# PufferAI/PufferLib

Hardware: AMD Instinct MI355X
Metric: env steps/sec end-to-end PPO (rollout+GAE+update), 4096 envs (higher is better)
Workload: dtype f32; 1 GPU; squared d=3 nt=1, 4096 envs/GPU x 128 steps, obs 49->64 f32 rows, MLP 128, 4 minibatches x 4 epochs, bptt 16 (BASELINE configs[1]); global_batch=524288, parallelism=dp1

## Files before the change

include/pufferlib_amd.h:

```cpp
#ifndef PUFFERLIB_AMD_H
#define PUFFERLIB_AMD_H
#include <stddef.h>
#include <stdint.h>

#ifdef __cplusplus
extern "C" {
#endif

typedef void *pfa_stream_t;

int pfa_version(void);
const char *pfa_last_error(void);

int pfa_timing_enable(int mode);
int pfa_timing_select(const char *kernel);
int pfa_timing_stride(int every);
int pfa_timing_reset(void);
int pfa_timing_read(const char *kernel, int64_t *launches_host, double *total_ms_host);

size_t pfa_gae_workspace_bytes(int64_t n);
int pfa_gae_f32(const float *dones, const float *values, const float *rewards, float *advantages,
                float *returns, int64_t n, float gamma, float gae_lambda, void *workspace,
                pfa_stream_t stream);
int pfa_gae_sums_supported(int64_t n, int32_t num_envs, int32_t num_minibatches, int32_t bptt_horizon);
size_t pfa_gae_sums_workspace_bytes(int64_t n, int32_t num_minibatches);
int pfa_gae_sums_f32(const float *dones, const float *values, const float *rewards, float *advantages, float *returns,
                     int64_t n, float gamma, float gae_lambda, int32_t num_envs, int32_t num_minibatches, int32_t bptt_horizon,
                     double *adv_stats, double *ev4, double *zero8, void *workspace, pfa_stream_t stream);
int32_t pfa_gae_halo_rows(float gamma, float gae_lambda);
int pfa_gae_halo_publish(const float *dones, const float *values, const float *rewards, int64_t n, float gamma, float gae_lambda,
                         const double *extra, int32_t n_extra, double *out, int32_t rank, int32_t world, pfa_stream_t stream);
int pfa_gae_halo_unpack(const double *gathered, int32_t rank, int32_t world, int64_t n, float gamma, float gae_lambda, float *dones,
                        float *values, float *rewards, pfa_stream_t stream);
int pfa_gae_halo_f32(const float *dones, const float *values, const float *rewards, float *advantages, float *returns, int64_t n,
                     int32_t halo_len, float gamma, float gae_lambda, int32_t num_envs, int32_t num_minibatches, int32_t bptt_horizon,
                     double *adv_stats, double *ev4, double *zero8, void *workspace, pfa_stream_t stream);
int pfa_gae_shard_pass2(const float *dones, const float *values, const float *rewards, float *advantages,
                        float *returns, int64_t n, int has_next, float gamma, float gae_lambda,
                        const void *workspace, const double *carry_in, pfa_stream_t stream);
int pfa_gae_shard_publish(const float *dones, const float *values, const float *rewards, int64_t n, float gamma, float gae_lambda,
                          void *workspace, const double *extra, int32_t n_extra, double *out, int32_t rank, int32_t world,
                          pfa_stream_t stream);
int pfa_gae_shard_fold(const double *gathered, int32_t rank, int32_t world, int64_t n, float gamma, float gae_lambda, void *workspace,
                       float *dones, float *values, float *rewards, double *carry_out, pfa_stream_t stream);


typedef struct {
    int32_t num_envs;
    int32_t distance_to_target;
    int32_t num_targets;
    int32_t obs_stride;
    int32_t tape_rounds;
} pfa_squared_config;

size_t pfa_squared_state_bytes(const pfa_squared_config *cfg);
int pfa_squared_async_reset(void *state, const pfa_squared_config *cfg, int64_t seed, float *obs,
                            float *rewards, uint8_t *terminals, uint8_t *truncations, uint8_t *masks,
                            pfa_stream_t stream);
int pfa_squared_fill_tape(void *state, const pfa_squared_config *cfg, int32_t rounds, pfa_stream_t stream);
int pfa_squared_send(void *state, const pfa_squared_config *cfg, const int64_t *actions, float *obs,
                     float *rewards, uint8_t *terminals, uint8_t *truncations, uint8_t *masks,
// ... 481 lines not shown
```

pufferlib_amd/_lib.py:

```python
import ctypes as C
import os
import subprocess

from .exceptions import ExtensionError

HERE = os.path.dirname(os.path.abspath(__file__))
REPO = os.path.dirname(HERE)
CSRC = os.path.join(HERE, 'csrc')
LIB_DIR = os.path.join(HERE, '_lib')
LIB_PATH = os.path.join(LIB_DIR, 'libpufferlib_amd.so')
SOURCES = ['common.cpp', 'dist.cpp', 'p2p.hip', 'gae.hip', 'squared.hip', 'pixel_squared.hip', 'rollout.hip', 'ppo_update.hip', 'lstm.hip', 'gemm.hip', 'lstm_fused.hip', 'lstm_seq.hip', 'stochastic.hip', 'memory.hip', 'bandit.hip', 'multiagent.hip', 'spaces.hip', 'synthetic.hip', 'tabular.hip', 'cartpole.hip', 'acrobot.hip', 'nativize.hip', 'igemm.hip', 'cnn_heads.hip', 'general.hip', 'ppo_wide.hip']
HEADERS = sorted(f for f in os.listdir(CSRC) if f.endswith('.hpp')) + [os.path.join('..', '..', 'include', 'pufferlib_amd.h')]


def _stale():
    if not os.path.exists(LIB_PATH):
        return True
    t = os.path.getmtime(LIB_PATH)
    deps = [os.path.join(CSRC, f) for f in SOURCES + HEADERS]
    return any(os.path.exists(d) and os.path.getmtime(d) > t for d in deps)


def source_hash():
    import hashlib
# ... 114 lines not shown


class Experience(C.Structure):
    _fields_ = [('obs', C.c_void_p), ('actions', C.c_void_p), ('logprobs', C.c_void_p), ('values', C.c_void_p),
                ('rewards', C.c_void_p), ('dones', C.c_void_p), ('advantages', C.c_void_p), ('returns', C.c_void_p),
                ('horizon_T', C.c_int32)]


class ReduceJob(C.Structure):
    _fields_ = [('kind', C.c_int32), ('splits', C.c_int32), ('mo', C.c_int32), ('no', C.c_int32), ('partial', C.c_void_p), ('c', C.c_void_p),
                ('ldc', C.c_int64), ('c2', C.c_void_p), ('ldc2', C.c_int64), ('nb', C.c_int32), ('reserved', C.c_int32)]


class PpoHparams(C.Structure):
    _fields_ = [('clip_coef', C.c_float), ('vf_clip_coef', C.c_float), ('vf_coef', C.c_float), ('ent_coef', C.c_float),
                ('norm_adv', C.c_int32), ('clip_vloss', C.c_int32), ('num_minibatches', C.c_int32),
                ('bptt_horizon', C.c_int32)]


P = C.c_void_p
_SIGNATURES = {
    'pfa_version': (C.c_int, []),
    'pfa_last_error': (C.c_char_p, []),
    'pfa_timing_enable': (C.c_int, [C.c_int]),
    'pfa_timing_select': (C.c_int, [C.c_char_p]),
    'pfa_timing_stride': (C.c_int, [C.c_int]),
    'pfa_timing_reset': (C.c_int, []),
    'pfa_timing_read': (C.c_int, [C.c_char_p, C.POINTER(C.c_int64), C.POINTER(C.c_double)]),
    'pfa_gae_workspace_bytes': (C.c_size_t, [C.c_int64]),
    'pfa_gae_f32': (C.c_int, [P, P, P, P, P, C.c_int64, C.c_float, C.c_float, P, P]),
    'pfa_gae_sums_supported': (C.c_int, [C.c_int64, C.c_int32, C.c_int32, C.c_int32]),
    'pfa_gae_sums_workspace_bytes': (C.c_size_t, [C.c_int64, C.c_int32]),
    'pfa_gae_sums_f32': (C.c_int, [P, P, P, P, P, C.c_int64, C.c_float, C.c_float, C.c_int32, C.c_int32, C.c_int32, P, P, P, P, P]),
    'pfa_gae_halo_rows': (C.c_int32, [C.c_float, C.c_float]),
    'pfa_gae_halo_publish': (C.c_int, [P, P, P, C.c_int64, C.c_float, C.c_float, P, C.c_int32, P, C.c_int32, C.c_int32, P]),
    'pfa_gae_halo_unpack': (C.c_int, [P, C.c_int32, C.c_int32, C.c_int64, C.c_float, C.c_float, P, P, P, P]),
    'pfa_gae_halo_f32': (C.c_int, [P, P, P, P, P, C.c_int64, C.c_int32, C.c_float, C.c_float, C.c_int32, C.c_int32, C.c_int32, P, P, P, P, P]),
    'pfa_gae_shard_pass2': (C.c_int, [P, P, P, P, P, C.c_int64, C.c_int, C.c_float, C.c_float, P, P, P]),
    'pfa_gae_shard_publish': (C.c_int, [P, P, P, C.c_int64, C.c_float, C.c_float, P, P, C.c_int32, P, C.c_int32, C.c_int32, P]),
    'pfa_gae_shard_fold': (C.c_int, [P, C.c_int32, C.c_int32, C.c_int64, C.c_float, C.c_float, P, P, P, P, P, P]),
    'pfa_train_ev_sums': (C.c_int, [C.POINTER(Experience), C.c_int64, C.c_int32, P, P, P]),
    'pfa_train_log_pack': (C.c_int, [P, P, P, P]),
    'pfa_squared_state_bytes': (C.c_size_t, [C.POINTER(SquaredConfig)]),
    'pfa_squared_async_reset': (C.c_int, [P, C.POINTER(SquaredConfig), C.c_int64, P, P, P, P, P, P]),
    'pfa_squared_fill_tape': (C.c_int, [P, C.POINTER(SquaredConfig), C.c_int32, P]),
    'pfa_squared_send': (C.c_int, [P, C.POINTER(SquaredConfig), P, P, P, P, P, P, P]),
    'pfa_squared_episode_stats': (C.c_int, [P, C.POINTER(SquaredConfig), P, C.c_int32, P]),
    'pfa_squared_last_infos': (C.c_int, [P, C.POINTER(SquaredConfig), P, P, P, P, P]),
    'pfa_squared_debug_targets': (C.c_int, [P, C.POINTER(SquaredConfig), P, P]),
    'pfa_squared_debug_stream_pos': (C.c_int, [P, C.POINTER(SquaredConfig), P, P]),
    'pfa_pixel_squared_state_bytes': (C.c_size_t, [C.POINTER(SquaredConfig), C.POINTER(PixelConfig)]),
    'pfa_pixel_squared_async_reset': (C.c_int, [P, C.POINTER(SquaredConfig), C.POINTER(PixelConfig), C.c_int64, P, P, P, P, P, P]),
    'pfa_pixel_squared_send': (C.c_int, [P, C.POINTER(SquaredConfig), C.POINTER(PixelConfig), P, P, P, P, P, P, P]),
    'pfa_mlp_param_count': (C.c_int64, [C.POINTER(MlpDims)]),
    'pfa_mlp_forward_sample': (C.c_int, [P, C.c_int64, P, C.POINTER(MlpDims), P, C.POINTER(NoiseKey), C.c_int64,
                                         P, P, P, P, P]),
    'pfa_philox_exp_noise': (C.c_int, [P, C.c_int64, C.c_int64, C.c_int32, C.POINTER(NoiseKey), C.c_int64, P]),
    'pfa_rollout_mlp_squared': (C.c_int, [P, C.POINTER(SquaredConfig), P, C.POINTER(MlpDims), C.POINTER(Experience),
                                          P, C.POINTER(NoiseKey), C.c_int64, P, P, P, P, P, P]),
    'pfa_mlp_view_supported': (C.c_int, [C.POINTER(MlpView)]),
    'pfa_ppo_wide_supported': (C.c_int, [C.POINTER(MlpView)]),
    'pfa_ppo_wide_workspace_bytes': (C.c_size_t, [C.POINTER(MlpView)]),
    'pfa_ppo_wide_grad': (C.c_int, [C.POINTER(Experience), C.c_int64, C.c_int32, C.POINTER(MlpView), C.POINTER(MlpView), P, C.POINTER(PpoHparams), P,
                                    C.c_int64, P, P]),
    'pfa_mlp_view_forward_sample': (C.c_int, [P, C.c_int64, C.POINTER(MlpView), P, C.POINTER(NoiseKey), C.c_int64, P, P, P, P, P]),
    'pfa_rollout_mlp_view_squared': (C.c_int, [P, C.POINTER(SquaredConfig), C.POINTER(MlpView), C.POINTER(Experience), P, C.POINTER(NoiseKey),
# ... 227 lines not shown
```

pufferlib_amd/clean_pufferl.py:

```python
import ctypes as C
import os
import random
import time
from collections import deque
from threading import Thread

import numpy as np
import torch

from . import _lib, readback, utils
from . import dist as pdist
from .cleanrl import Policy, RecurrentPolicy, _weights_changed, reads_frames, route
from .models import FlatParams
from .namespace import namespace
from .vector import Frames, PixelSquared, Spaces, Squared, Stochastic, _DeviceVecEnv


def seed_everything(seed, torch_deterministic=True):
    random.seed(seed)
    np.random.seed(seed)
    if seed is not None:
        torch.manual_seed(seed)
    torch.backends.cudnn.deterministic = torch_deterministic

# ... 526 lines not shown
            data._gae_done = _gae_key(data)
        if readback.eager():
            data._rb_eval.resolve()
    return stats, infos


def _early_gae():
    return os.environ.get('PFA_EARLY_GAE', '1') != '0'


def _ev_with_gae(data, world):
    return not (getattr(data, 'arrival_values', None) is not None and _cfg(data.config, 'async_store', 'balanced') == 'reference')


def _fused_sums_ok(data, world=1):
    config, experience = data.config, data.experience
    return (_ev_with_gae(data, world)
            and bool(_lib.lib().pfa_gae_sums_supported(experience.batch_size, experience.num_envs, experience.num_minibatches,
                                                       int(config.bptt_horizon))))


def _gae_key(data):
    config, ex = data.config, data.experience
    rdv = getattr(ex, '_rdv', None)
    ver = rdv._version if rdv is not None else (ex.rewards._version, ex.dones._version, ex.values._version)
    ptrs = tuple(int(getattr(ex, k).data_ptr()) for k in ('rewards', 'dones', 'values', 'advantages', 'returns'))
    return (ver, ptrs, ex.batch_size, float(config.gamma), float(config.gae_lambda), ex.num_envs, ex.num_minibatches,
            int(config.bptt_horizon), bool(config.norm_adv))


def _launch_gae_sums(data):
    config, experience = data.config, data.experience
    nmb = experience.num_minibatches
    _lib.check(_lib.lib().pfa_gae_sums_f32(
        _lib.ptr(experience.dones), _lib.ptr(experience.values), _lib.ptr(experience.rewards), _lib.ptr(experience.advantages),
        _lib.ptr(experience.returns), experience.batch_size, float(config.gamma), float(config.gae_lambda), experience.num_envs, nmb,
        int(config.bptt_horizon), _lib.ptr(data.adv_stats), C.c_void_p(data.dp_sums.data_ptr() + 16 * nmb), _lib.ptr(data.loss_acc),
        _lib.ptr(data.workspace), _lib.stream_handle()), 'gae_sums')


def _all_reduce(data, buf, what):
    if data.native_dp:
        L = _lib.lib()
        fn = L.pfa_dist_all_reduce_f64 if buf.dtype == torch.float64 else L.pfa_dist_all_reduce_f32
        _lib.check(fn(_lib.ptr(buf), buf.numel(), _lib.stream_handle()), what)
    elif data.world_size > 1:
        _dist()[0].all_reduce(buf)


def _publish_gae(data, extra=None):
    config, ex = data.config, data.experience
    L, B, stream = _lib.lib(), ex.batch_size, _lib.stream_handle()
    _, rank, world = _dist()
    gamma, lam = float(config.gamma), float(config.gae_lambda)
    n_extra = 0 if extra is None else extra.numel()
    H = int(L.pfa_gae_halo_rows(gamma, lam))
    if getattr(ex, '_rdv', None) is None or ex._rdv.shape[1] < B + H:
        H = 0
    size = n_extra + (3 * world * min(B, H) if H else 6 * world)
    if data._dp_eval is None or data._dp_eval.numel() != size:
        data._dp_eval = torch.zeros(size, dtype=torch.float64, device=ex.device)
    buf = data._dp_eval
    rows = (_lib.ptr(ex.dones), _lib.ptr(ex.values), _lib.ptr(ex.rewards))
    if H:
        _lib.check(L.pfa_gae_halo_publish(*rows, B, gamma, lam, _lib.ptr(extra), n_extra, _lib.ptr(buf), rank, world, stream), 'gae halo publish')
    else:
        _lib.check(L.pfa_gae_shard_publish(*rows, B, gamma, lam, _lib.ptr(data.gae_ws), _lib.ptr(extra), n_extra, _lib.ptr(buf), rank, world,
                                           stream), 'gae publish')
    _all_reduce(data, buf, 'stats + gae all-reduce')
    data._gae_published = (H, n_extra)
    return buf[:n_extra]
# ... 310 lines not shown
```

pufferlib_amd/csrc/gae.hip:

```cpp
#include <cmath>
#include <cstdlib>

#include "common.hpp"

#define PFA_GAE_FP _Pragma("clang fp contract(off)")

namespace pfa {

constexpr int kGaeThreads = 256;
constexpr int kGaeItems = 8;
constexpr int kGaeBlock = kGaeThreads * kGaeItems;

struct Affine {
    double c, d;
};

__device__ __forceinline__ Affine compose(const Affine &outer, const Affine &inner) {
    return {outer.c * inner.c, outer.d + outer.c * inner.d};
}

__device__ __forceinline__ Affine shfl_down_affine(const Affine &a, int off) {
    return {__shfl_down(a.c, off, 64), __shfl_down(a.d, off, 64)};
}

struct GaeItems {
    float v[kGaeItems + 1], r[kGaeItems + 1], d[kGaeItems + 1];
};

__device__ __forceinline__ void gae_load(const float *dones, const float *values, const float *rewards, long long s,
                                         long long n, GaeItems &it) {
#pragma unroll
    for (int i = 0; i <= kGaeItems; ++i) {
        const long long t = s + i;
        const bool ok = t < n;
        it.v[i] = ok ? values[t] : 0.0f;
        it.r[i] = ok ? rewards[t] : 0.0f;
        it.d[i] = ok ? dones[t] : 0.0f;
    }
}

__device__ __forceinline__ Affine gae_thread_map(const GaeItems &it, long long s, long long n, float gamma, float lam,
                                                 bool pin_last) {
    PFA_GAE_FP
    Affine f = {1.0, 0.0};
#pragma unroll
    for (int i = kGaeItems - 1; i >= 0; --i) {
        const long long t = s + i;
        if (t >= n) continue;
        if (t == n - 1 && pin_last) {
            f = {0.0, 0.0};
            continue;
        }
        const float nnt = 1.0f - it.d[i + 1];
        const float delta = (it.r[i + 1] + (gamma * it.v[i + 1]) * nnt) - it.v[i];
        const float coef = (gamma * lam) * nnt;
        f = compose({(double)coef, (double)delta}, f);
    }
    return f;
}

template <int NT = kGaeThreads>
__device__ __forceinline__ void block_suffix_scan(Affine &mine, Affine &after, Affine *sh) {
    const int lane = lane_id(), wv = wave_id();
// ... 48 lines not shown
        if (lane == 0) s_carry = f.c * (carry_in ? *carry_in : 0.0) + f.d;
    }
    const long long s = (long long)blockIdx.x * kGaeBlock + (long long)threadIdx.x * kGaeItems;
    GaeItems it;
    gae_load(dones, values, rewards, s, n + halo, it);
    Affine mine = gae_thread_map(it, s, n, gamma, lam, halo == 0), after;
    block_suffix_scan(mine, after, sh);
    float last = (float)(after.c * s_carry + after.d);
    {
    PFA_GAE_FP
#pragma unroll
    for (int i = kGaeItems - 1; i >= 0; --i) {
        const long long t = s + i;
        if (t >= n) continue;
        if (t == n - 1 && halo == 0) {
            last = 0.0f;
        } else {
            const float nnt = 1.0f - it.d[i + 1];
            const float delta = (it.r[i + 1] + (gamma * it.v[i + 1]) * nnt) - it.v[i];
            last = delta + ((gamma * lam) * nnt) * last;
        }
        adv[t] = last;
        if (ret) ret[t] = last + it.v[i];
    }
    }
}

constexpr int kGaeChunkThreads = 128;
constexpr int kGaeChunk = kGaeChunkThreads * kGaeItems;
struct GaeSums {
    double *part;
    int nmb, bptt;
    int num_envs, horizon;
};
template <bool SUMS, bool SELF, int CT = kGaeChunkThreads>
__global__ void __launch_bounds__(2 * CT) gae_exact_kernel(const float *dones, const float *values, const float *rewards, float *adv,
                                                               float *ret, long long n, long long n_read, float gamma, float lam,
                                                               const Affine *agg, int nchunks, int warm, GaeSums sums) {
    constexpr int kChunk = CT * kGaeItems, kWin = 2 * kChunk, kNT = 2 * CT;
    __shared__ Affine sh[SELF ? 1 : kNT / 64];
    __shared__ double s_carry;
    __shared__ float2 cd[kWin + kWin / 8];
    __shared__ float start[SELF ? 1 : kNT];
    __shared__ double sh_s[SUMS ? 4 : 1][SUMS ? CT : 1];
    const int tid = threadIdx.x;
    if (!SELF && wave_id() == 0) {
        const int first = blockIdx.x + 2, cnt = nchunks - first;
        const int per = cnt > 0 ? (cnt + 63) / 64 : 0;
        const int lane = lane_id();
        Affine f = {1.0, 0.0};
        for (int i = per - 1; i >= 0; --i) {
            const int b = first + lane * per + i;
            if (b < nchunks) f = compose(agg[b], f);
        }
#pragma unroll
        for (int off = 1; off < 64; off <<= 1) {
            const Affine o = shfl_down_affine(f, off);
            if (lane + off < 64) f = compose(f, o);
        }
        if (lane == 0) s_carry = f.d;
    }
    const long long s = (long long)blockIdx.x * kChunk + (long long)tid * kGaeItems;
    GaeItems it;
    const bool feeds = !SELF || tid * kGaeItems < kChunk + kGaeItems + warm;
    if (feeds) gae_load(dones, values, rewards, s, n_read, it);
    if constexpr (!SELF) {
        Affine mine = gae_thread_map(it, s, n, gamma, lam, true), after;
        block_suffix_scan<kNT>(mine, after, sh);
        start[tid] = (float)(after.c * s_carry + after.d);
    }
    if (feeds) {
    PFA_GAE_FP
#pragma unroll
    for (int i = 0; i < kGaeItems; ++i) {
        const long long t = s + i;
        float2 e = make_float2(0.0f, 0.0f);
        if (t < n_read - 1) {
            const float nnt = 1.0f - it.d[i + 1];
            e.y = (it.r[i + 1] + (gamma * it.v[i + 1]) * nnt) - it.v[i];
            e.x = (gamma * lam) * nnt;
        }
        const int li = tid * kGaeItems + i;
        cd[li + (li >> 3)] = e;
    }
    }
    __syncthreads();
    float advv[kGaeItems];
#pragma unroll
    for (int i = 0; i < kGaeItems; ++i) advv[i] = 0.0f;
    if (tid < CT) {
        PFA_GAE_FP
        const int first = tid * kGaeItems + kGaeItems;
        float x = SELF ? 0.0f : start[tid + (warm >> 3)];
        for (int li = first + warm - kGaeItems; li >= first; li -= kGaeItems) {
            const float2 *grp = cd + li + (li >> 3);
            float2 e[kGaeItems];
#pragma unroll
            for (int k = 0; k < kGaeItems; ++k) e[k] = grp[k];
#pragma unroll
            for (int k = kGaeItems - 1; k >= 0; --k) x = e[k].y + e[k].x * x;
        }
#pragma unroll
        for (int i = kGaeItems - 1; i >= 0; --i) {
            const int li = tid * kGaeItems + i;
            const float2 e = cd[li + (li >> 3)];
            x = e.y + e.x * x;
            advv[i] = x;
            const long long t = s + i;
            if (t < n) {
                adv[t] = x;
                if (ret) ret[t] = x + it.v[i];
            }
        }
    }
    if constexpr (SUMS) {
        double a1 = 0.0, a2 = 0.0, y1 = 0.0, y2 = 0.0;
        if (tid < CT) {
            float yp[kGaeItems];
            const long long e0 = s % sums.num_envs, t0 = s / sums.num_envs;
#pragma unroll
            for (int i = 0; i < kGaeItems; ++i) {
                long long e = e0 + i, t = t0;
                while (e >= sums.num_envs) {
                    e -= sums.num_envs;
                    ++t;
                }
                yp[i] = s + i < n ? values[e * sums.horizon + t] : 0.0f;
            }
#pragma unroll
            for (int i = 0; i < kGaeItems; ++i) {
                if (s + i >= n) continue;
                const double a = (double)advv[i], y = a + (double)yp[i];
                a1 += a;
                a2 += a * a;
                y1 += y;
                y2 += y * y;
            }
            sh_s[0][tid] = a1;
            sh_s[1][tid] = a2;
            sh_s[2][tid] = y1;
            sh_s[3][tid] = y2;
        }
        __syncthreads();
        const int G = sums.bptt / kGaeItems, P = G * sums.nmb;
        for (int stride = CT / 2; stride >= P; stride >>= 1) {
            if (tid < stride) {
#pragma unroll
                for (int q = 0; q < 4; ++q) sh_s[q][tid] += sh_s[q][tid + stride];
            }
            __syncthreads();
        }
        double *out = sums.part + (size_t)blockIdx.x * (2 * sums.nmb + 4);
        if (tid < 2 * sums.nmb) {
            const int m = tid >> 1, k = tid & 1;
            double v = 0.0;
            for (int g = 0; g < G; ++g) v += sh_s[k][m * G + g];
            out[tid] = v;
        } else if (tid >= 64 && tid < 68) {
            const int k = tid - 64, src = k < 2 ? 2 + k : k - 2;
            double v = 0.0;
            for (int g = 0; g < P; ++g) v += sh_s[src][g];
            out[2 * sums.nmb + k] = v;
        }
    }
}

__global__ void __launch_bounds__(64) gae_sums_final_kernel(const double *part, int nblocks, int nmb, double *adv_stats, double *ev4, double *zero8) {
    const int q = blockIdx.x, lane = threadIdx.x, width = 2 * nmb + 4;
    double v = 0.0;
    for (int b = lane; b < nblocks; b += 64) v += part[(size_t)b * width + q];
#pragma unroll
    for (int o = 32; o > 0; o >>= 1) v += __shfl_xor(v, o, 64);
    if (lane == 0) {
        if (q < 2 * nmb) adv_stats[q] = v;
        else ev4[q - 2 * nmb] = v;
    }
    if (q == 0 && zero8 && lane < 8) zero8[lane] = 0.0;
}

__global__ void gae_shard_publish_kernel(const Affine *agg, int nblocks, const float *dones, const float *values, const float *rewards,
                                         long long n, const double *extra, int n_extra, double *out, int rank, int world) {
    const int lane = lane_id();
    const int per = (nblocks + 63) / 64;
    Affine f = {1.0, 0.0};
    for (int i = per - 1; i >= 0; --i) {
        const int b = lane * per + i;
        if (b < nblocks) f = compose(agg[b], f);
    }
#pragma unroll
    for (int off = 1; off < 64; off <<= 1) {
        const Affine o = shfl_down_affine(f, off);
        if (lane + off < 64) f = compose(f, o);
    }
    const double c = __shfl(f.c, 0, 64), d = __shfl(f.d, 0, 64);
    for (int i = lane; i < n_extra; i += 64) out[i] = extra[i];
    for (int i = lane; i < 6 * world; i += 64) {
// ... 108 lines not shown
    if (n == 0) return 0;
    PFA_REQUIRE(dones && values && rewards && advantages && workspace, "gae: null buffer");
    const int64_t nc = (n + kGaeChunk - 1) / kGaeChunk;
    PFA_REQUIRE(nc <= 0x7fffffff, "gae: batch too large");
    Affine *agg = (Affine *)workspace;
    ScopedKernelTimer timer("gae", (hipStream_t)stream);
    if (const int ws = gae_warm_self(gamma, gae_lambda)) {
        launch_gae_self<false>(dones, values, rewards, advantages, returns, n, n, gamma, gae_lambda, ws, GaeSums{}, (hipStream_t)stream);
        PFA_LAUNCH_CHECK();
        return 0;
    }
    hipLaunchKernelGGL(gae_aggregate_kernel<kGaeChunkThreads>, dim3((unsigned)nc), dim3(kGaeChunkThreads), 0, (hipStream_t)stream, dones, values,
                       rewards, (long long)n, gamma, gae_lambda, agg, 0);
    PFA_LAUNCH_CHECK();
    hipLaunchKernelGGL((gae_exact_kernel<false, false>), dim3((unsigned)nc), dim3(kGaeThreads), 0, (hipStream_t)stream, dones, values, rewards,
                       advantages, returns, (long long)n, (long long)n, gamma, gae_lambda, agg, (int)nc, gae_warm(gamma, gae_lambda), GaeSums{});
    PFA_LAUNCH_CHECK();
    return 0;
}

static bool gae_sums_ok(int64_t n, int num_envs, int nmb, int bptt) {
    if (n < 1 || num_envs < 1 || nmb < 1 || bptt < kGaeItems || bptt % kGaeItems) return false;
    if (n % num_envs || n % ((int64_t)nmb * bptt)) return false;
    const int64_t P = (int64_t)(bptt / kGaeItems) * nmb;
    return P <= kGaeChunkThreads && (P & (P - 1)) == 0 && 2 * nmb <= 64;
}
extern "C" int pfa_gae_sums_supported(int64_t n, int32_t num_envs, int32_t num_minibatches, int32_t bptt_horizon) {
    return gae_sums_ok(n, num_envs, num_minibatches, bptt_horizon) ? 1 : 0;
}
extern "C" size_t pfa_gae_sums_workspace_bytes(int64_t n, int32_t num_minibatches) {
    const int64_t nc = (n + kGaeChunk - 1) / kGaeChunk;
    return align_up((size_t)(nc > 0 ? nc : 1) * sizeof(Affine), 256) + (size_t)(nc > 0 ? nc : 1) * (2 * (size_t)num_minibatches + 4) * sizeof(double);
}
extern "C" int pfa_gae_sums_f32(const float *dones, const float *values, const float *rewards, float *advantages, float *returns,
                                int64_t n, float gamma, float gae_lambda, int32_t num_envs, int32_t num_minibatches, int32_t bptt_horizon,
                                double *adv_stats, double *ev4, double *zero8, void *workspace, pfa_stream_t stream) {
    PFA_REQUIRE(gae_sums_ok(n, num_envs, num_minibatches, bptt_horizon), "gae_sums: unsupported partition (pfa_gae_sums_supported)");
    PFA_REQUIRE(dones && values && rewards && advantages && adv_stats && ev4 && workspace, "gae_sums: null buffer");
    const int64_t nc = (n + kGaeChunk - 1) / kGaeChunk;
    PFA_REQUIRE(nc <= 0x7fffffff, "gae: batch too large");
    Affine *agg = (Affine *)workspace;
    GaeSums sums{(double *)((char *)workspace + align_up((size_t)nc * sizeof(Affine), 256)), num_minibatches, bptt_horizon, num_envs,
                 (int)(n / num_envs)};
    ScopedKernelTimer timer("gae", (hipStream_t)stream);
    int64_t nparts = nc;
    if (const int ws = gae_warm_self(gamma, gae_lambda)) {
        nparts = launch_gae_self<true>(dones, values, rewards, advantages, returns, n, n, gamma, gae_lambda, ws, sums, (hipStream_t)stream);
    } else {
        hipLaunchKernelGGL(gae_aggregate_kernel<kGaeChunkThreads>, dim3((unsigned)nc), dim3(kGaeChunkThreads), 0, (hipStream_t)stream, dones, values,
                           rewards, (long long)n, gamma, gae_lambda, agg, 0);
        PFA_LAUNCH_CHECK();
        hipLaunchKernelGGL((gae_exact_kernel<true, false>), dim3((unsigned)nc), dim3(kGaeThreads), 0, (hipStream_t)stream, dones, values, rewards,
                           advantages, returns, (long long)n, (long long)n, gamma, gae_lambda, agg, (int)nc, gae_warm(gamma, gae_lambda), sums);
    }
    PFA_LAUNCH_CHECK();
    hipLaunchKernelGGL(gae_sums_final_kernel, dim3((unsigned)(2 * num_minibatches + 4)), dim3(64), 0, (hipStream_t)stream, sums.part, (int)nparts,
                       (int)num_minibatches, adv_stats, ev4, zero8);
    PFA_LAUNCH_CHECK();
    return 0;
}

extern "C" int pfa_gae_shard_pass2(const float *dones, const float *values, const float *rewards, float *advantages,
                                   float *returns, int64_t n, int has_next, float gamma, float gae_lambda,
                                   const void *workspace, const double *carry_in, pfa_stream_t stream) {
    PFA_REQUIRE(n >= 1 && dones && values && rewards && advantages && workspace, "gae_shard: bad arguments");
    PFA_REQUIRE(!has_next || carry_in, "gae_shard: a shard with a successor needs carry_in");
    const int64_t nb = (n + kGaeBlock - 1) / kGaeBlock;
    hipLaunchKernelGGL(gae_apply_kernel, dim3((unsigned)nb), dim3(kGaeThreads), 0, (hipStream_t)stream, dones, values, rewards,
                       advantages, returns, (long long)n, gamma, gae_lambda, (const Affine *)workspace, (int)nb,
                       has_next ? carry_in : (const double *)nullptr, has_next ? 1 : 0);
    PFA_LAUNCH_CHECK();
    return 0;
}

extern "C" int pfa_gae_shard_publish(const float *dones, const float *values, const float *rewards, int64_t n, float gamma, float gae_lambda,
                                     void *workspace, const double *extra, int32_t n_extra, double *out, int32_t rank, int32_t world,
                                     pfa_stream_t stream) {
    PFA_REQUIRE(n >= 1 && dones && values && rewards && workspace && out && world >= 1 && rank >= 0 && rank < world && n_extra >= 0 &&
                    (n_extra == 0 || extra),
                "gae_shard_publish: bad arguments");
    const int64_t nb = (n + kGaeBlock - 1) / kGaeBlock;
    PFA_REQUIRE(nb <= 0x7fffffff, "gae: batch too large");
    Affine *agg = (Affine *)workspace;
    hipLaunchKernelGGL(gae_aggregate_kernel<kGaeThreads>, dim3((unsigned)nb), dim3(kGaeThreads), 0, (hipStream_t)stream, dones, values, rewards,
                       (long long)(n - 1), gamma, gae_lambda, agg, 1);
    PFA_LAUNCH_CHECK();
    hipLaunchKernelGGL(gae_shard_publish_kernel, dim3(1), dim3(64), 0, (hipStream_t)stream, agg, (int)nb, dones, values, rewards, (long long)n,
                       extra, (int)n_extra, out, (int)rank, (int)world);
    PFA_LAUNCH_CHECK();
    return 0;
}

// ... 37 lines not shown
    const int len = gae_halo_len(n, rank, world, H);
    if (len > 0) {
        hipLaunchKernelGGL(gae_halo_unpack_kernel, dim3((unsigned)((len + 255) / 256)), dim3(256), 0, (hipStream_t)stream, gathered,
                           (int)(n < H ? n : H), (int)rank, (long long)n, len, dones, values, rewards);
        PFA_LAUNCH_CHECK();
    }
    return len;
}
extern "C" int pfa_gae_halo_f32(const float *dones, const float *values, const float *rewards, float *advantages, float *returns, int64_t n,
                                int32_t halo_len, float gamma, float gae_lambda, int32_t num_envs, int32_t num_minibatches, int32_t bptt_horizon,
                                double *adv_stats, double *ev4, double *zero8, void *workspace, pfa_stream_t stream) {
    const int ws = gae_warm_self(gamma, gae_lambda);
    PFA_REQUIRE(ws > 0, "gae_halo: gamma * lambda = %g is outside the self-starting window (pfa_gae_halo_rows)", (double)(gamma * gae_lambda));
    PFA_REQUIRE(n >= 1 && halo_len >= 0 && halo_len <= ws + kGaeItems && dones && values && rewards && advantages, "gae_halo: bad arguments");
    const int64_t nc = (n + kGaeChunk - 1) / kGaeChunk;
    PFA_REQUIRE(nc <= 0x7fffffff, "gae: batch too large");
    ScopedKernelTimer timer("gae", (hipStream_t)stream);
    if (!adv_stats) {
        launch_gae_self<false>(dones, values, rewards, advantages, returns, n, n + halo_len, gamma, gae_lambda, ws, GaeSums{}, (hipStream_t)stream);
        PFA_LAUNCH_CHECK();
        return 0;
    }
    PFA_REQUIRE(gae_sums_ok(n, num_envs, num_minibatches, bptt_horizon), "gae_halo: unsupported partition for the sums (pfa_gae_sums_supported)");
    PFA_REQUIRE(ev4 && workspace, "gae_halo: null buffer");
    GaeSums sums{(double *)((char *)workspace + align_up((size_t)nc * sizeof(Affine), 256)), num_minibatches, bptt_horizon, num_envs,
                 (int)(n / num_envs)};
    const int64_t nparts = launch_gae_self<true>(dones, values, rewards, advantages, returns, n, n + halo_len, gamma, gae_lambda, ws, sums, (hipStream_t)stream);
    PFA_LAUNCH_CHECK();
    hipLaunchKernelGGL(gae_sums_final_kernel, dim3((unsigned)(2 * num_minibatches + 4)), dim3(64), 0, (hipStream_t)stream, sums.part, (int)nparts,
                       (int)num_minibatches, adv_stats, ev4, zero8);
    PFA_LAUNCH_CHECK();
    return 0;
}
```

pufferlib_amd/csrc/squared.hip:

```cpp
#include "common.hpp"
#include "mt19937.hpp"
#include "squared_env.hpp"

namespace pfa {

struct Sampler {
    int n, k, i;
    bool pool_path;
    uint8_t picks[kMaxTargets];
    uint8_t ov_pos[kMaxTargets];
    uint8_t ov_val[kMaxTargets];

    __device__ void begin(int n_, int k_) {
        n = n_;
        k = k_;
        i = 0;
        int setsize = 21;
        if (k > 5) {
            int p = 1;
            while (p < 3 * k) p *= 4;
            setsize += p;
        }
        pool_path = n <= setsize;
    }
// ... 316 lines not shown
                v.tape[(size_t)(round % v.tape_rounds) * v.n + env] = (uint16_t)perimeter_cell((int)cand[i], v.g);
                if (pos == job.need - 1) s_last = p0 + i;
            }
            ++pos;
        }
    }
    __syncthreads();
    const long long last = s_last;
    if (last >= 0) {
        const long long consumed = last + 1, at = job.idx0 + consumed;
        long long blk = at / kMtN;
        int idx = (int)(at % kMtN);
        if (idx == 0 && blk > 0) { blk -= 1; idx = kMtN; }
        for (int i = tid; i < kMtN; i += kSelThreads) v.hdr->mt[i] = raw[blk * kMtN + i];
        if (tid == 0) {
            v.hdr->mt_idx = idx;
            v.hdr->words += (unsigned long long)consumed;
            v.hdr->rounds_filled = job.first_round + rounds;
        }
    } else if (tail && before + total < job.need && tid == 0) {
        v.hdr->underrun = 1;
    }
}

__global__ void __launch_bounds__(256) squared_send_kernel(SquaredView v, const long long *actions, float *obs,
                                                          float *rewards, uint8_t *terminals, uint8_t *truncations,
                                                          uint8_t *masks) {
    const int e = blockIdx.x * blockDim.x + threadIdx.x;
    if (e >= v.n) return;
    uint16_t tc[kMaxTargets];
    squared_send_env(v, e, (int)actions[e], obs + (size_t)e * v.stride, tc, rewards, terminals, truncations, masks);
}

__global__ void __launch_bounds__(256) squared_stats_kernel(SquaredView v, double *out4, int reset) {
    __shared__ double sh[4][256];
    double a[4] = {0, 0, 0, 0};
    constexpr int kBatch = 8;
    int e0 = threadIdx.x;
    for (; e0 + 256 * (kBatch - 1) < v.n; e0 += 256 * kBatch) {
        int cnt[kBatch];
        long long len[kBatch];
        double ret[kBatch], score[kBatch];
#pragma unroll
        for (int k = 0; k < kBatch; ++k) {
            const int e = e0 + 256 * k;
            cnt[k] = v.acc_cnt[e];
            ret[k] = v.acc_ret[e];
            len[k] = v.acc_len[e];
            score[k] = v.acc_score[e];
        }
#pragma unroll
        for (int k = 0; k < kBatch; ++k) {
            const int e = e0 + 256 * k;
            a[0] += (double)cnt[k];
            a[1] += ret[k];
            a[2] += (double)len[k];
            a[3] += score[k];
            if (reset) {
                v.acc_cnt[e] = 0;
                v.acc_ret[e] = 0.0;
                v.acc_len[e] = 0;
                v.acc_score[e] = 0.0;
            }
        }
    }
    for (int e = e0; e < v.n; e += 256) {
        a[0] += (double)v.acc_cnt[e];
        a[1] += v.acc_ret[e];
        a[2] += (double)v.acc_len[e];
        a[3] += v.acc_score[e];
        if (reset) {
            v.acc_cnt[e] = 0;
            v.acc_ret[e] = 0.0;
            v.acc_len[e] = 0;
            v.acc_score[e] = 0.0;
        }
    }
    for (int q = 0; q < 4; ++q) sh[q][threadIdx.x] = a[q];
    __syncthreads();
    for (int s = 128; s > 0; s >>= 1) {
        if ((int)threadIdx.x < s)
            for (int q = 0; q < 4; ++q) sh[q][threadIdx.x] += sh[q][threadIdx.x + s];
        __syncthreads();
    }
    if (threadIdx.x < 4) out4[threadIdx.x] = sh[threadIdx.x][0];
    if (threadIdx.x == 4) out4[4] = (double)v.hdr->underrun;
}

__global__ void squared_infos_kernel(SquaredView v, uint8_t *fin, double *ret, int32_t *len, double *score) {
    const int e = blockIdx.x * blockDim.x + threadIdx.x;
    if (e >= v.n) return;
    fin[e] = v.fin[e];
    ret[e] = v.fin_ret[e];
    len[e] = v.fin_len[e];
    score[e] = v.fin_score[e];
}

__global__ void squared_debug_targets_kernel(SquaredView v, int32_t *cells) {
    const int e = blockIdx.x * blockDim.x + threadIdx.x;
    if (e >= v.n) return;
    const uint32_t rem = v.rem[e];
    for (int t = 0; t < v.nt; ++t) cells[(size_t)e * v.nt + t] = ((rem >> t) & 1u) ? (int)v.tgt[(size_t)t * v.n + e] : -1;
}

__global__ void squared_debug_pos_kernel(SquaredView v, unsigned long long *pos) { *pos = v.hdr->words; }

static int check_cfg(const pfa_squared_config *c) {
    PFA_REQUIRE(c != nullptr, "squared: null config");
    PFA_REQUIRE(c->num_envs >= 1, "squared: num_envs must be at least 1");
    PFA_REQUIRE(c->distance_to_target >= 1 && c->distance_to_target <= 15, "squared: distance_to_target must be in 1..15");
    PFA_REQUIRE(c->num_targets >= 1 && c->num_targets <= kMaxTargets && c->num_targets <= 8 * c->distance_to_target,
                "squared: num_targets must be in 1..min(32, 8*distance_to_target)");
    const int g = 2 * c->distance_to_target + 1;
    PFA_REQUIRE(c->obs_stride >= g * g, "squared: obs_stride %d < grid cells %d", c->obs_stride, g * g);
    PFA_REQUIRE(c->tape_rounds >= 1, "squared: tape_rounds must be >= 1");
    return 0;
}

}
// ... 75 lines not shown
    hipLaunchKernelGGL(squared_stats_kernel, dim3(1), dim3(256), 0, (hipStream_t)stream, v, out4, (int)reset);
    PFA_LAUNCH_CHECK();
    return 0;
}

extern "C" int pfa_squared_last_infos(void *state, const pfa_squared_config *cfg, uint8_t *finished, double *episode_return,
                                      int32_t *episode_length, double *score, pfa_stream_t stream) {
    if (int rc = check_cfg(cfg)) return rc;
    PFA_REQUIRE(state && finished && episode_return && episode_length && score, "squared.last_infos: null buffer");
    SquaredView v = squared_view(state, *cfg);
    const int blocks = (cfg->num_envs + 255) / 256;
    hipLaunchKernelGGL(squared_infos_kernel, dim3(blocks), dim3(256), 0, (hipStream_t)stream, v, finished, episode_return,
                       episode_length, score);
    PFA_LAUNCH_CHECK();
    return 0;
}

extern "C" int pfa_squared_debug_targets(void *state, const pfa_squared_config *cfg, int32_t *cells, pfa_stream_t stream) {
    if (int rc = check_cfg(cfg)) return rc;
    SquaredView v = squared_view(state, *cfg);
    const int blocks = (cfg->num_envs + 255) / 256;
    hipLaunchKernelGGL(squared_debug_targets_kernel, dim3(blocks), dim3(256), 0, (hipStream_t)stream, v, cells);
    PFA_LAUNCH_CHECK();
    return 0;
}

extern "C" int pfa_squared_debug_stream_pos(void *state, const pfa_squared_config *cfg, uint64_t *pos_device, pfa_stream_t stream) {
    if (int rc = check_cfg(cfg)) return rc;
    SquaredView v = squared_view(state, *cfg);
    hipLaunchKernelGGL(squared_debug_pos_kernel, dim3(1), dim3(1), 0, (hipStream_t)stream, v, (unsigned long long *)pos_device);
    PFA_LAUNCH_CHECK();
    return 0;
}
```

Measured before the change: 434.3 million env_steps/s.

## Fuse GAE sums finalization into one launch and vectorize GAE loads/stores

Adds a last-block-done ticket so the GAE self-warm kernel folds the per-block partial sums itself, removing the separate finalize launch. The change also vectorizes GAE loads and stores with float4, issues the value gather early, software-pipelines the LDS scan loop, and rewrites the squared stats reduction to use wave shuffles with a separate reset pass. Probe timestamp macros are added behind a compile flag. In exchange it adds a cached per-workspace ticket allocation, a serial tail in the last block, and atomic ordering assumptions.

Measured after the change: 434.0 million env_steps/s. No clear change (-0.1%).

```diff
diff --git a/include/pufferlib_amd.h b/include/pufferlib_amd.h
--- a/include/pufferlib_amd.h
+++ b/include/pufferlib_amd.h
@@ -27,6 +27,10 @@
 int pfa_gae_sums_f32(const float *dones, const float *values, const float *rewards, float *advantages, float *returns,
                      int64_t n, float gamma, float gae_lambda, int32_t num_envs, int32_t num_minibatches, int32_t bptt_horizon,
                      double *adv_stats, double *ev4, double *zero8, void *workspace, pfa_stream_t stream);
+int pfa_gae_sums_launches_f32(const float *dones, const float *values, const float *rewards, float *advantages, float *returns,
+                              int64_t n, float gamma, float gae_lambda, int32_t num_envs, int32_t num_minibatches,
+                              int32_t bptt_horizon, double *adv_stats, double *ev4, double *zero8, void *workspace,
+                              int32_t one_launch, pfa_stream_t stream);
 int32_t pfa_gae_halo_rows(float gamma, float gae_lambda);
 int pfa_gae_halo_publish(const float *dones, const float *values, const float *rewards, int64_t n, float gamma, float gae_lambda,
                          const double *extra, int32_t n_extra, double *out, int32_t rank, int32_t world, pfa_stream_t stream);
diff --git a/pufferlib_amd/_lib.py b/pufferlib_amd/_lib.py
--- a/pufferlib_amd/_lib.py
+++ b/pufferlib_amd/_lib.py
@@ -170,6 +170,7 @@
     'pfa_gae_sums_supported': (C.c_int, [C.c_int64, C.c_int32, C.c_int32, C.c_int32]),
     'pfa_gae_sums_workspace_bytes': (C.c_size_t, [C.c_int64, C.c_int32]),
     'pfa_gae_sums_f32': (C.c_int, [P, P, P, P, P, C.c_int64, C.c_float, C.c_float, C.c_int32, C.c_int32, C.c_int32, P, P, P, P, P]),
+    'pfa_gae_sums_launches_f32': (C.c_int, [P, P, P, P, P, C.c_int64, C.c_float, C.c_float, C.c_int32, C.c_int32, C.c_int32, P, P, P, P, C.c_int32, P]),
     'pfa_gae_halo_rows': (C.c_int32, [C.c_float, C.c_float]),
     'pfa_gae_halo_publish': (C.c_int, [P, P, P, C.c_int64, C.c_float, C.c_float, P, C.c_int32, P, C.c_int32, C.c_int32, P]),
     'pfa_gae_halo_unpack': (C.c_int, [P, C.c_int32, C.c_int32, C.c_int64, C.c_float, C.c_float, P, P, P, P]),
diff --git a/pufferlib_amd/clean_pufferl.py b/pufferlib_amd/clean_pufferl.py
--- a/pufferlib_amd/clean_pufferl.py
+++ b/pufferlib_amd/clean_pufferl.py
@@ -582,11 +582,11 @@
 def _launch_gae_sums(data):
     config, experience = data.config, data.experience
     nmb = experience.num_minibatches
-    _lib.check(_lib.lib().pfa_gae_sums_f32(
+    _lib.check(_lib.lib().pfa_gae_sums_launches_f32(
         _lib.ptr(experience.dones), _lib.ptr(experience.values), _lib.ptr(experience.rewards), _lib.ptr(experience.advantages),
         _lib.ptr(experience.returns), experience.batch_size, float(config.gamma), float(config.gae_lambda), experience.num_envs, nmb,
         int(config.bptt_horizon), _lib.ptr(data.adv_stats), C.c_void_p(data.dp_sums.data_ptr() + 16 * nmb), _lib.ptr(data.loss_acc),
-        _lib.ptr(data.workspace), _lib.stream_handle()), 'gae_sums')
+        _lib.ptr(data.workspace), 1, _lib.stream_handle()), 'gae_sums')
 
 
 def _all_reduce(data, buf, what):
diff --git a/pufferlib_amd/csrc/gae.hip b/pufferlib_amd/csrc/gae.hip
--- a/pufferlib_amd/csrc/gae.hip
+++ b/pufferlib_amd/csrc/gae.hip
@@ -1,5 +1,6 @@
 #include <cmath>
 #include <cstdlib>
+#include <unordered_map>
 
 #include "common.hpp"
 
@@ -29,6 +30,18 @@
 
 __device__ __forceinline__ void gae_load(const float *dones, const float *values, const float *rewards, long long s,
                                          long long n, GaeItems &it) {
+    if (s + kGaeItems < n && (((size_t)dones | (size_t)values | (size_t)rewards) & 15) == 0) {
+        const float *src[3] = {values, rewards, dones};
+        float *dst[3] = {it.v, it.r, it.d};
+#pragma unroll
+        for (int a = 0; a < 3; ++a) {
+            const float4 lo = *(const float4 *)(src[a] + s), hi = *(const float4 *)(src[a] + s + 4);
+            dst[a][0] = lo.x, dst[a][1] = lo.y, dst[a][2] = lo.z, dst[a][3] = lo.w;
+            dst[a][4] = hi.x, dst[a][5] = hi.y, dst[a][6] = hi.z, dst[a][7] = hi.w;
+            dst[a][8] = src[a][s + kGaeItems];
+        }
+        return;
+    }
 #pragma unroll
     for (int i = 0; i <= kGaeItems; ++i) {
         const long long t = s + i;
@@ -143,7 +156,58 @@
     double *part;
     int nmb, bptt;
     int num_envs, horizon;
+    unsigned *ticket;
+    double *adv_stats, *ev4, *zero8;
 };
+
+#ifdef PFA_PROBES
+__device__ unsigned long long *g_gae_trace = nullptr;
+__device__ int g_gae_trace_block = 0;
+#define PFA_GSTAMP(k)                                                                                               \
+    do {                                                                                                            \
+        if (g_gae_trace && (int)blockIdx.x == g_gae_trace_block && (threadIdx.x & 63) == 0)                         \
+            g_gae_trace[(size_t)(threadIdx.x >> 6) * 8 + (k)] = __builtin_amdgcn_s_memtime();                       \
+    } while (0)
+#else
+#define PFA_GSTAMP(k) do { } while (0)
+#endif
+
+__device__ __forceinline__ void part_store(double *p, double v) {
+    __hip_atomic_store((unsigned long long *)p, (unsigned long long)__double_as_longlong(v), __ATOMIC_RELAXED, __HIP_MEMORY_SCOPE_AGENT);
+}
+__device__ __forceinline__ unsigned long long part_load(const double *p) {
+    return __hip_atomic_load((const unsigned long long *)p, __ATOMIC_RELAXED, __HIP_MEMORY_SCOPE_AGENT);
+}
+
+template <int Q>
+__device__ __forceinline__ void gae_final_sums(const double *part, int nblocks, int width, int q0, int qs, int lane, double (&v)[Q]) {
+    constexpr int KB = 8;
+#pragma unroll
+    for (int j = 0; j < Q; ++j) v[j] = 0.0;
+    for (int b0 = lane; b0 < nblocks; b0 += 64 * KB) {
+        unsigned long long x[Q][KB];
+#pragma unroll
+        for (int j = 0; j < Q; ++j) {
+#pragma unroll
+            for (int k = 0; k < KB; ++k) {
+                const int q = q0 + j * qs, b = b0 + 64 * k;
+                x[j][k] = q < width && b < nblocks ? part_load(part + (size_t)b * width + q) : 0ull;
+            }
+        }
+#pragma unroll
+        for (int j = 0; j < Q; ++j) {
+#pragma unroll
+            for (int k = 0; k < KB; ++k) {
+                if (q0 + j * qs < width && b0 + 64 * k < nblocks) v[j] += __longlong_as_double((long long)x[j][k]);
+            }
+        }
+    }
+#pragma unroll
+    for (int j = 0; j < Q; ++j) {
+#pragma unroll
+        for (int o = 32; o > 0; o >>= 1) v[j] += __shfl_xor(v[j], o, 64);
+    }
+}
 template <bool SUMS, bool SELF, int CT = kGaeChunkThreads>
 __global__ void __launch_bounds__(2 * CT) gae_exact_kernel(const float *dones, const float *values, const float *rewards, float *adv,
                                                                float *ret, long long n, long long n_read, float gamma, float lam,
@@ -174,7 +238,23 @@
     const long long s = (long long)blockIdx.x * kChunk + (long long)tid * kGaeItems;
     GaeItems it;
     const bool feeds = !SELF || tid * kGaeItems < kChunk + kGaeItems + warm;
+    PFA_GSTAMP(0);
     if (feeds) gae_load(dones, values, rewards, s, n_read, it);
+    long long gat[SUMS ? kGaeItems : 1];
+    if constexpr (SUMS) {
+        if (tid < CT) {
+            const long long e0 = s % sums.num_envs, t0 = s / sums.num_envs;
+#pragma unroll
+            for (int i = 0; i < kGaeItems; ++i) {
+                long long e = e0 + i, t = t0;
+                while (e >= sums.num_envs) {
+                    e -= sums.num_envs;
+                    ++t;
+                }
+                gat[i] = e * sums.horizon + t;
+            }
+        }
+    }
     if constexpr (!SELF) {
         Affine mine = gae_thread_map(it, s, n, gamma, lam, true), after;
         block_suffix_scan<kNT>(mine, after, sh);
@@ -195,49 +275,82 @@
         cd[li + (li >> 3)] = e;
     }
     }
+    float yp[SUMS ? kGaeItems : 1];
+    if constexpr (SUMS) {
+        __builtin_amdgcn_s_waitcnt(0x0f70);
+        if (tid < CT) {
+#pragma unroll
+            for (int i = 0; i < kGaeItems; ++i) yp[i] = s + i < n ? values[gat[i]] : 0.0f;
+        }
+    }
+    PFA_GSTAMP(1);
     __syncthreads();
+    PFA_GSTAMP(2);
     float advv[kGaeItems];
 #pragma unroll
     for (int i = 0; i < kGaeItems; ++i) advv[i] = 0.0f;
     if (tid < CT) {
         PFA_GAE_FP
-        const int first = tid * kGaeItems + kGaeItems;
+        const int own = tid * kGaeItems;
         float x = SELF ? 0.0f : start[tid + (warm >> 3)];
-        for (int li = first + warm - kGaeItems; li >= first; li -= kGaeItems) {
+        const auto load = [&](float2 (&e)[kGaeItems], int li) {
             const float2 *grp = cd + li + (li >> 3);
-            float2 e[kGaeItems];
 #pragma unroll
             for (int k = 0; k < kGaeItems; ++k) e[k] = grp[k];
+        };
+        const auto steps = [&](const float2 (&e)[kGaeItems]) {
 #pragma unroll
             for (int k = kGaeItems - 1; k >= 0; --k) x = e[k].y + e[k].x * x;
-        }
+        };
+        float2 ea[kGaeItems], eb[kGaeItems];
+        int li = own + warm;
+        load(ea, li);
+        for (; li >= own + 2 * kGaeItems; li -= 2 * kGaeItems) {
+            load(eb, li - kGaeItems);
+            __builtin_amdgcn_sched_barrier(0);
+            steps(ea);
+            __builtin_amdgcn_sched_barrier(0);
+            load(ea, li - 2 * kGaeItems);
+            __builtin_amdgcn_sched_barrier(0);
+            steps(eb);
+            __builtin_amdgcn_sched_barrier(0);
+        }
+        if (li > own) {
+            load(eb, own);
+            __builtin_amdgcn_sched_barrier(0);
+            steps(ea);
+            __builtin_amdgcn_sched_barrier(0);
+#pragma unroll
+            for (int k = 0; k < kGaeItems; ++k) ea[k] = eb[k];
+        }
+        PFA_GSTAMP(3);
 #pragma unroll
         for (int i = kGaeItems - 1; i >= 0; --i) {
-            const int li = tid * kGaeItems + i;
-            const float2 e = cd[li + (li >> 3)];
-            x = e.y + e.x * x;
+            x = ea[i].y + ea[i].x * x;
             advv[i] = x;
-            const long long t = s + i;
-            if (t < n) {
-                adv[t] = x;
-                if (ret) ret[t] = x + it.v[i];
+        }
+        if (s + kGaeItems <= n && (((size_t)adv | (size_t)ret) & 15) == 0) {
+            *(float4 *)(adv + s) = make_float4(advv[0], advv[1], advv[2], advv[3]);
+            *(float4 *)(adv + s + 4) = make_float4(advv[4], advv[5], advv[6], advv[7]);
+            if (ret) {
+                *(float4 *)(ret + s) = make_float4(advv[0] + it.v[0], advv[1] + it.v[1], advv[2] + it.v[2], advv[3] + it.v[3]);
+                *(float4 *)(ret + s + 4) = make_float4(advv[4] + it.v[4], advv[5] + it.v[5], advv[6] + it.v[6], advv[7] + it.v[7]);
             }
-        }
-    }
+        } else {
+#pragma unroll
+            for (int i = 0; i < kGaeItems; ++i) {
+                const long long t = s + i;
+                if (t < n) {
+                    adv[t] = advv[i];
+                    if (ret) ret[t] = advv[i] + it.v[i];
+                }
+            }
+        }
+    }
+    PFA_GSTAMP(4);
     if constexpr (SUMS) {
         double a1 = 0.0, a2 = 0.0, y1 = 0.0, y2 = 0.0;
         if (tid < CT) {
-            float yp[kGaeItems];
-            const long long e0 = s % sums.num_envs, t0 = s / sums.num_envs;
-#pragma unroll
-            for (int i = 0; i < kGaeItems; ++i) {
-                long long e = e0 + i, t = t0;
-                while (e >= sums.num_envs) {
-                    e -= sums.num_envs;
-                    ++t;
-                }
-                yp[i] = s + i < n ? values[e * sums.horizon + t] : 0.0f;
-            }
 #pragma unroll
             for (int i = 0; i < kGaeItems; ++i) {
                 if (s + i >= n) continue;
@@ -261,18 +374,47 @@
             }
             __syncthreads();
         }
-        double *out = sums.part + (size_t)blockIdx.x * (2 * sums.nmb + 4);
+        PFA_GSTAMP(5);
+        const int width = 2 * sums.nmb + 4;
+        double *out = sums.part + (size_t)blockIdx.x * width;
         if (tid < 2 * sums.nmb) {
             const int m = tid >> 1, k = tid & 1;
             double v = 0.0;
             for (int g = 0; g < G; ++g) v += sh_s[k][m * G + g];
-            out[tid] = v;
+            part_store(out + tid, v);
         } else if (tid >= 64 && tid < 68) {
             const int k = tid - 64, src = k < 2 ? 2 + k : k - 2;
             double v = 0.0;
             for (int g = 0; g < P; ++g) v += sh_s[src][g];
-            out[2 * sums.nmb + k] = v;
-        }
+            part_store(out + 2 * sums.nmb + k, v);
+        }
+        PFA_GSTAMP(6);
+        if (sums.ticket) {
+            __shared__ int s_last;
+            asm volatile("s_waitcnt vmcnt(0)" ::: "memory");
+            __syncthreads();
+            if (tid == 0) s_last = __hip_atomic_fetch_add(sums.ticket, 1u, __ATOMIC_RELAXED, __HIP_MEMORY_SCOPE_AGENT) == gridDim.x - 1;
+            __syncthreads();
+            if (s_last) {
+                constexpr int Q = 4;
+                const int lane = lane_id(), wv = wave_id(), nw = kNT / 64;
+                for (int q0 = wv; q0 < width; q0 += Q * nw) {
+                    double v[Q];
+                    gae_final_sums<Q>(sums.part, (int)gridDim.x, width, q0, nw, lane, v);
+#pragma unroll
+                    for (int j = 0; j < Q; ++j) {
+                        const int q = q0 + j * nw;
+                        if (lane == 0 && q < width) {
+                            if (q < 2 * sums.nmb) sums.adv_stats[q] = v[j];
+                            else sums.ev4[q - 2 * sums.nmb] = v[j];
+                        }
+                    }
+                }
+                if (sums.zero8 && tid < 8) sums.zero8[tid] = 0.0;
+                if (tid == 0) __hip_atomic_store(sums.ticket, 0u, __ATOMIC_RELAXED, __HIP_MEMORY_SCOPE_AGENT);
+            }
+        }
+        PFA_GSTAMP(7);
     }
 }
 
@@ -447,9 +589,29 @@
     const int64_t nc = (n + kGaeChunk - 1) / kGaeChunk;
     return align_up((size_t)(nc > 0 ? nc : 1) * sizeof(Affine), 256) + (size_t)(nc > 0 ? nc : 1) * (2 * (size_t)num_minibatches + 4) * sizeof(double);
 }
-extern "C" int pfa_gae_sums_f32(const float *dones, const float *values, const float *rewards, float *advantages, float *returns,
-                                int64_t n, float gamma, float gae_lambda, int32_t num_envs, int32_t num_minibatches, int32_t bptt_horizon,
-                                double *adv_stats, double *ev4, double *zero8, void *workspace, pfa_stream_t stream) {
+static unsigned *gae_ticket_of(void *workspace) {
+    static std::unordered_map<void *, unsigned *> words;
+    auto it = words.find(workspace);
+    if (it != words.end()) return it->second;
+    if (words.size() >= 64) {
+        (void)hipDeviceSynchronize();
+        for (auto &kv : words) (void)hipFree(kv.second);
+        words.clear();
+    }
+    void *p = nullptr;
+    if (hipMalloc(&p, 256) != hipSuccess) return nullptr;
+    if (hipMemset(p, 0, 256) != hipSuccess || hipDeviceSynchronize() != hipSuccess) {
+        (void)hipFree(p);
+        return nullptr;
+    }
+    words[workspace] = (unsigned *)p;
+    return (unsigned *)p;
+}
+
+extern "C" int pfa_gae_sums_launches_f32(const float *dones, const float *values, const float *rewards, float *advantages, float *returns,
+                                         int64_t n, float gamma, float gae_lambda, int32_t num_envs, int32_t num_minibatches,
+                                         int32_t bptt_horizon, double *adv_stats, double *ev4, double *zero8, void *workspace,
+                                         int32_t one_launch, pfa_stream_t stream) {
     PFA_REQUIRE(gae_sums_ok(n, num_envs, num_minibatches, bptt_horizon), "gae_sums: unsupported partition (pfa_gae_sums_supported)");
     PFA_REQUIRE(dones && values && rewards && advantages && adv_stats && ev4 && workspace, "gae_sums: null buffer");
     const int64_t nc = (n + kGaeChunk - 1) / kGaeChunk;
@@ -457,10 +619,22 @@
     Affine *agg = (Affine *)workspace;
     GaeSums sums{(double *)((char *)workspace + align_up((size_t)nc * sizeof(Affine), 256)), num_minibatches, bptt_horizon, num_envs,
                  (int)(n / num_envs)};
+    const int ws = gae_warm_self(gamma, gae_lambda);
+    if (one_launch && ws) {
+        sums.ticket = gae_ticket_of(workspace);
+        PFA_REQUIRE(sums.ticket, "gae_sums: cannot allocate the ticket word");
+        sums.adv_stats = adv_stats;
+        sums.ev4 = ev4;
+        sums.zero8 = zero8;
+    }
     ScopedKernelTimer timer("gae", (hipStream_t)stream);
     int64_t nparts = nc;
-    if (const int ws = gae_warm_self(gamma, gae_lambda)) {
+    if (ws) {
         nparts = launch_gae_self<true>(dones, values, rewards, advantages, returns, n, n, gamma, gae_lambda, ws, sums, (hipStream_t)stream);
+        if (sums.ticket) {
+            PFA_LAUNCH_CHECK();
+            return 0;
+        }
     } else {
         hipLaunchKernelGGL(gae_aggregate_kernel<kGaeChunkThreads>, dim3((unsigned)nc), dim3(kGaeChunkThreads), 0, (hipStream_t)stream, dones, values,
                            rewards, (long long)n, gamma, gae_lambda, agg, 0);
@@ -473,6 +647,13 @@
                        (int)num_minibatches, adv_stats, ev4, zero8);
     PFA_LAUNCH_CHECK();
     return 0;
+}
+
+extern "C" int pfa_gae_sums_f32(const float *dones, const float *values, const float *rewards, float *advantages, float *returns,
+                                int64_t n, float gamma, float gae_lambda, int32_t num_envs, int32_t num_minibatches, int32_t bptt_horizon,
+                                double *adv_stats, double *ev4, double *zero8, void *workspace, pfa_stream_t stream) {
+    return pfa_gae_sums_launches_f32(dones, values, rewards, advantages, returns, n, gamma, gae_lambda, num_envs, num_minibatches, bptt_horizon,
+                                     adv_stats, ev4, zero8, workspace, 1, stream);
 }
 
 extern "C" int pfa_gae_shard_pass2(const float *dones, const float *values, const float *rewards, float *advantages,
@@ -576,3 +757,10 @@
     PFA_LAUNCH_CHECK();
     return 0;
 }
+
+#ifdef PFA_PROBES
+extern "C" int pfa_probe_set_gae_trace(unsigned long long *trace, int block) {
+    if (hipMemcpyToSymbol(HIP_SYMBOL(g_gae_trace), &trace, sizeof(trace)) != hipSuccess) return 1;
+    return hipMemcpyToSymbol(HIP_SYMBOL(g_gae_trace_block), &block, sizeof(block)) == hipSuccess ? 0 : 1;
+}
+#endif
diff --git a/pufferlib_amd/csrc/squared.hip b/pufferlib_amd/csrc/squared.hip
--- a/pufferlib_amd/csrc/squared.hip
+++ b/pufferlib_amd/csrc/squared.hip
@@ -372,59 +372,83 @@
     squared_send_env(v, e, (int)actions[e], obs + (size_t)e * v.stride, tc, rewards, terminals, truncations, masks);
 }
 
+#ifdef PFA_PROBES
+__device__ unsigned long long *g_stats_trace = nullptr;
+#define PFA_SSTAMP(k)                                                                          \
+    do {                                                                                       \
+        if (g_stats_trace && threadIdx.x == 0) g_stats_trace[k] = __builtin_amdgcn_s_memtime(); \
+    } while (0)
+#else
+#define PFA_SSTAMP(k) do { } while (0)
+#endif
+
+template <int kBatch>
+__device__ __forceinline__ void squared_stats_batch(const SquaredView &v, int e0, double (&a)[4]) {
+    int cnt[kBatch];
+    long long len[kBatch];
+    double ret[kBatch], score[kBatch];
+#pragma unroll
+    for (int k = 0; k < kBatch; ++k) {
+        const int e = e0 + 256 * k;
+        cnt[k] = v.acc_cnt[e];
+        ret[k] = v.acc_ret[e];
+        len[k] = v.acc_len[e];
+        score[k] = v.acc_score[e];
+    }
+#pragma unroll
+    for (int k = 0; k < kBatch; ++k) {
+        a[0] += (double)cnt[k];
+        a[1] += ret[k];
+        a[2] += (double)len[k];
+        a[3] += score[k];
+    }
+}
+
 __global__ void __launch_bounds__(256) squared_stats_kernel(SquaredView v, double *out4, int reset) {
     __shared__ double sh[4][256];
     double a[4] = {0, 0, 0, 0};
-    constexpr int kBatch = 8;
+    PFA_SSTAMP(0);
+    const int underrun = v.hdr->underrun;
     int e0 = threadIdx.x;
-    for (; e0 + 256 * (kBatch - 1) < v.n; e0 += 256 * kBatch) {
-        int cnt[kBatch];
-        long long len[kBatch];
-        double ret[kBatch], score[kBatch];
-#pragma unroll
-        for (int k = 0; k < kBatch; ++k) {
-            const int e = e0 + 256 * k;
-            cnt[k] = v.acc_cnt[e];
-            ret[k] = v.acc_ret[e];
-            len[k] = v.acc_len[e];
-            score[k] = v.acc_score[e];
-        }
-#pragma unroll
-        for (int k = 0; k < kBatch; ++k) {
-            const int e = e0 + 256 * k;
-            a[0] += (double)cnt[k];
-            a[1] += ret[k];
-            a[2] += (double)len[k];
-            a[3] += score[k];
-            if (reset) {
-                v.acc_cnt[e] = 0;
-                v.acc_ret[e] = 0.0;
-                v.acc_len[e] = 0;
-                v.acc_score[e] = 0.0;
-            }
-        }
-    }
+    for (; e0 + 256 * 15 < v.n; e0 += 256 * 16) squared_stats_batch<16>(v, e0, a);
+    for (; e0 + 256 * 7 < v.n; e0 += 256 * 8) squared_stats_batch<8>(v, e0, a);
     for (int e = e0; e < v.n; e += 256) {
         a[0] += (double)v.acc_cnt[e];
         a[1] += v.acc_ret[e];
         a[2] += (double)v.acc_len[e];
         a[3] += v.acc_score[e];
-        if (reset) {
+    }
+    PFA_SSTAMP(1);
+    for (int q = 0; q < 4; ++q) sh[q][threadIdx.x] = a[q];
+    __syncthreads();
+    PFA_SSTAMP(2);
+    if (threadIdx.x < 64) {
+        const int t = threadIdx.x;
+        double r[4];
+#pragma unroll
+        for (int q = 0; q < 4; ++q) r[q] = (sh[q][t] + sh[q][t + 128]) + (sh[q][t + 64] + sh[q][t + 192]);
+#pragma unroll
+        for (int s = 32; s > 0; s >>= 1) {
+#pragma unroll
+            for (int q = 0; q < 4; ++q) r[q] += __shfl_down(r[q], s, 64);
+        }
+        PFA_SSTAMP(3);
+        if (t == 0) {
+#pragma unroll
+            for (int q = 0; q < 4; ++q) out4[q] = r[q];
+            out4[4] = (double)underrun;
+        }
+        PFA_SSTAMP(4);
+    }
+    if (reset) {
+        for (int e = threadIdx.x; e < v.n; e += 256) {
             v.acc_cnt[e] = 0;
             v.acc_ret[e] = 0.0;
             v.acc_len[e] = 0;
             v.acc_score[e] = 0.0;
         }
     }
-    for (int q = 0; q < 4; ++q) sh[q][threadIdx.x] = a[q];
-    __syncthreads();
-    for (int s = 128; s > 0; s >>= 1) {
-        if ((int)threadIdx.x < s)
-            for (int q = 0; q < 4; ++q) sh[q][threadIdx.x] += sh[q][threadIdx.x + s];
-        __syncthreads();
-    }
-    if (threadIdx.x < 4) out4[threadIdx.x] = sh[threadIdx.x][0];
-    if (threadIdx.x == 4) out4[4] = (double)v.hdr->underrun;
+    PFA_SSTAMP(5);
 }
 
 __global__ void squared_infos_kernel(SquaredView v, uint8_t *fin, double *ret, int32_t *len, double *score) {
@@ -566,3 +590,9 @@
     PFA_LAUNCH_CHECK();
     return 0;
 }
+
+#ifdef PFA_PROBES
+extern "C" int pfa_probe_set_stats_trace(unsigned long long *trace) {
+    return hipMemcpyToSymbol(HIP_SYMBOL(pfa::g_stats_trace), &trace, sizeof(trace)) == hipSuccess ? 0 : 1;
+}
+#endif
```
